# NVIDIA/tensorrt-laboratory

Hardware: AMD Instinct MI355X
Metric: inferences/sec (higher is better)
Workload: dtype fp16; 1 GPU; model=resnet50, global_batch=8, batch_per_gpu=8, image=224, contexts=3, parallelism=dp1

## Files before the change

### csrc/kernels/conv.hip

```cpp
#include "conv_igemm.h"

namespace trtlab {

size_t conv_scratch_bytes(int Nb, int H, int W, int C, int Cout, int KH,
                          int KW, int sh, int sw, int ph, int pw) {
  int OH = (H + 2 * ph - KH) / sh + 1;
  int OW = (W + 2 * pw - KW) / sw + 1;
  int M = Nb * OH * OW;
  int K = (int)round_up(KH * KW * C, 64);
  TileCfg cfg = pick_tile(M, Cout);
  long tiles = cdiv(M, cfg.bm) * cdiv(Cout, cfg.bn);
  int splitk = pick_splitk(tiles, K >> 6);
  if (splitk == 1) return 0;
  return (size_t)tiles * splitk * cfg.bm * cfg.bn * 4;
}

template <typename T, int CM, bool DEEP, int BM = 64>
__global__ __launch_bounds__(256) void bottleneck_tail_kernel(
    const T* __restrict__ in, const T* __restrict__ W1,
    const T* __restrict__ W2, T* __restrict__ out,
    const float* __restrict__ s1, const float* __restrict__ b1,
    const float* __restrict__ s2, const float* __restrict__ b2,
    const T* __restrict__ residual, const T* __restrict__ zero_page,
    const ConvParams p, int Co) {
  constexpr int BNC = 64;
  constexpr int NB1 = CM / BNC;
  constexpr int kABytes = BM * 128;
  constexpr int kBuf = (BM + BNC) * 128;
  constexpr int NBUF = DEEP ? 4 : 2;
  constexpr int kT2 = CM / 64;
  constexpr int kTBlk = BM * 128;
  constexpr int kTBytes = kT2 * kTBlk;
  constexpr int kSmem =
      (NBUF * kBuf > kTBytes + 8192) ? NBUF * kBuf : kTBytes + 8192;
  __shared__ __attribute__((aligned(16))) char smem[kSmem];
  uint32_t lds0 = (uint32_t)(uintptr_t)&smem[0];

  uint32_t tile = xcd_swizzle(blockIdx.x, gridDim.x);
  int m0 = (int)tile * BM;
  const int tid = threadIdx.x;
  const int lane = tid & 63;
  const int wave = tid >> 6;
  const int wr = wave >> 1;
  const int wc = wave & 1;

  typename Mfma16x16x32<T>::accv acc1[NB1][BM / 32][BNC / 32];
#pragma unroll
  for (int c = 0; c < NB1; ++c)
#pragma unroll
    for (int i = 0; i < BM / 32; ++i)
#pragma unroll
      for (int j = 0; j < BNC / 32; ++j) acc1[c][i][j] = {0, 0, 0, 0};

  const int ktiles = p.K / kTileElems<T>;
  const TapRows<BM> rows = tap_rows_init<T, BM>(p, m0, tid);
  for (int nc = 0; nc < NB1; ++nc) {
    TapCursor tap = tap_cursor_init<T>(p, 0);
    auto stage1 = [&](int t, int slot) {
      uint32_t base = lds0 + slot * kBuf;
      stage_conv_a_tap<T, BM>(in, zero_page, p, rows, tap, base, tid);
      stage_tile<T, BNC, true>(W1 + (int64_t)nc * BNC * p.K +
                             (int64_t)t * kTileElems<T>,
                         p.K, nc * BNC, CM, base + kABytes, tid);
    };
    if constexpr (DEEP) {
      constexpr int G = BM / 32 + BNC / 32;
      for (int i = 0; i < 3 && i < ktiles; ++i) stage1(i, i);
      for (int t = 0; t < ktiles; ++t) {
        int ahead = ktiles - 1 - t;
        if (ahead > 2) ahead = 2;
        wait_tiles_inflight<G>(ahead);
        __builtin_amdgcn_s_barrier();
        if (t + 3 < ktiles) stage1(t + 3, (t + 3) & 3);
        const char* As = &smem[(t & 3) * kBuf];
        mfma_tile<T, BM, BNC, true>(As, As + kABytes, lane, wr, wc, acc1[nc]);
      }
      asm volatile("s_waitcnt vmcnt(0)" ::: "memory");
      __syncthreads();
    } else {
      stage1(0, 0);
      asm volatile("s_waitcnt vmcnt(0)" ::: "memory");
      __syncthreads();
      int cur = 0;
      for (int t = 0; t < ktiles; ++t) {
        if (t + 1 < ktiles) stage1(t + 1, cur ^ 1);
        const char* As = &smem[cur * kBuf];
        mfma_tile<T, BM, BNC, true>(As, As + kABytes, lane, wr, wc, acc1[nc]);
        asm volatile("s_waitcnt vmcnt(0)" ::: "memory");
        __syncthreads();
        cur ^= 1;
      }
    }
  }

  static_assert(BNC == 64 && sizeof(T) == 2, "one 16-B chunk per lane");
#pragma unroll
  for (int nc = 0; nc < NB1; ++nc) {
    const int col0 = nc * BNC + wc * (BNC / 2) + (lane >> 4) * 8;
    float sc[8], bi[8];
#pragma unroll
    for (int c = 0; c < 8; ++c) {
      sc[c] = s1[col0 + c];
      bi[c] = b1[col0 + c];
    }
#pragma unroll
    for (int i = 0; i < BM / 32; ++i) {
      uint32_t row = (uint32_t)(wr * (BM / 2) + i * 16 + (lane & 15));
      __attribute__((aligned(16))) T o[8];
#pragma unroll
      for (int j = 0; j < BNC / 32; ++j)
#pragma unroll
        for (int r = 0; r < 4; ++r)
          o[4 * j + r] = (T)fmaxf(
              (float)acc1[nc][i][j][r] * sc[4 * j + r] + bi[4 * j + r], 0.0f);
      uint32_t kb = (uint32_t)(col0 & 63) * (uint32_t)sizeof(T);
      uint32_t off = (uint32_t)(col0 >> 6) * (uint32_t)kTBlk + (row << 7) +
                     (kb ^ ((row & 7) << 4));
      i32x4 t;
      __builtin_memcpy(&t, o, 16);
      *(i32x4*)(smem + off) = t;
    }
  }
  __syncthreads();

  const char* Tlds = smem;
  char* B2s = smem + kTBytes;
  for (int c2 = 0; c2 < Co / 64; ++c2) {
#pragma unroll
    for (int t = 0; t < kT2; ++t)
      stage_tile<T, 64, true>(W2 + (int64_t)c2 * 64 * CM + t * kTileElems<T>, CM,
                        c2 * 64, Co, (uint32_t)(uintptr_t)(B2s + t * 8192),
                        tid);
    asm volatile("s_waitcnt vmcnt(0)" ::: "memory");
    __syncthreads();
    typename Mfma16x16x32<T>::accv acc2[BM / 32][2];
#pragma unroll
    for (int i = 0; i < BM / 32; ++i)
#pragma unroll
      for (int j = 0; j < 2; ++j) acc2[i][j] = {0, 0, 0, 0};
#pragma unroll
    for (int t = 0; t < kT2; ++t)
      mfma_tile<T, BM, 64, true>(Tlds + t * kTBlk, B2s + t * 8192, lane, wr, wc,
                           acc2);
    store_epilogue<T, Epi::kScaleBiasAddRelu, BM, 64>(
        acc2, out, Co, m0, c2 * 64, p.M, Co, s2, b2, residual, p.res_scale,
        lane, wr, wc);
    __syncthreads();
  }
}

void launch_bottleneck_tail(int dtype, const void* in, const void* W1,
                            const void* W2, void* out, const float* s1,
                            const float* b1, const float* s2, const float* b2,
                            const void* residual, const void* zero_page,
                            int Nb, int H, int W, int Cm, int Co,
                            hipStream_t stream) {
  if (dtype != 0)
    throw std::runtime_error("bottleneck_tail: fp16 only");
  if (Cm != 64 && Cm != 128)
    throw std::runtime_error("bottleneck_tail: Cm must be 64 or 128");
  if (Co % 64 != 0) throw std::runtime_error("bottleneck_tail: Co % 64");
  if (!tap_offsets_fit((int64_t)Nb * H * W * Cm * 2))
    throw std::runtime_error("bottleneck_tail: input must be under 2 GiB");
  ConvParams p;
  p.res_scale = 1.0f;
  p.Nb = Nb; p.H = H; p.W = W; p.C = Cm;
  p.Cout = Cm; p.KH = 3; p.KW = 3;
  p.sh = 1; p.sw = 1; p.ph = 1; p.pw = 1;
  p.OH = H; p.OW = W;
  p.M = Nb * H * W;
  p.Kreal = 9 * Cm;
  p.K = p.Kreal;
  p.d_ohw = make_fastdiv((uint32_t)(p.OH * p.OW));
  p.d_ow = make_fastdiv((uint32_t)p.OW);
  p.d_c = make_fastdiv((uint32_t)Cm);
  p.d_kw = make_fastdiv((uint32_t)p.KW);
  int bm = (cdiv(p.M, 64) >= 256) ? 64 : 32;
  dim3 grid((unsigned)cdiv(p.M, bm));
  bool deep = want_deep_pipe(grid.x, p.K / 64);
  auto go = [&](auto cm, auto dp, auto bmv) {
    constexpr int CMv = decltype(cm)::value;
    constexpr bool DPv = decltype(dp)::value;
    constexpr int BMv = decltype(bmv)::value;
    hipLaunchKernelGGL((bottleneck_tail_kernel<_Float16, CMv, DPv, BMv>),
                       grid, dim3(256), 0, stream, (const _Float16*)in,
                       (const _Float16*)W1, (const _Float16*)W2,
                       (_Float16*)out, s1, b1, s2, b2,
                       (const _Float16*)residual, (const _Float16*)zero_page,
                       p, Co);
  };
  auto c64 = std::integral_constant<int, 64>{};
  auto c128 = std::integral_constant<int, 128>{};
  auto b64 = std::integral_constant<int, 64>{};
  auto b32 = std::integral_constant<int, 32>{};
  if (Cm == 64) {
    if (bm == 64) { deep ? go(c64, std::true_type{}, b64)
                         : go(c64, std::false_type{}, b64); }
    else { deep ? go(c64, std::true_type{}, b32)
                : go(c64, std::false_type{}, b32); }
  } else {
// ... 63 lines not shown
```

### csrc/kernels/conv_igemm.h

```cpp
#pragma once
#include "gemm_common.h"

namespace trtlab {

struct ConvParams {
  int Nb, H, W, C;
  int Cout, KH, KW;
  int OH, OW;
  int sh, sw, ph, pw;
  int M;
  int K;
  int Kreal;
  float res_scale;
  FastDiv d_ohw, d_ow, d_c, d_kw;
};

template <typename T, int ROWS>
__device__ __forceinline__ void stage_conv_a(
    const T* __restrict__ in, const T* __restrict__ zero_page,
    const ConvParams p, int m0, int k0, uint32_t lds_base, int tid) {
#pragma unroll
  for (int c = 0; c < ROWS / 32; ++c) {
    uint32_t pbyte = c * 4096 + tid * 16;
    uint32_t row = pbyte >> 7;
// ... 115 lines not shown
void launch_splitk_reduce(int dtype, const float* scratch, void* C,
                          const float* scale, const float* bias,
                          const void* residual, float res_scale, int M, int N,
                          int64_t ldc, int tiles_m, int tiles_n, int splitk,
                          int bm, int bn, int epi, hipStream_t stream);

template <typename T, Epi E, int BM, int BN, bool SPLIT, int NBUF,
          bool TAP = false>
__global__ __launch_bounds__(256) void conv_igemm_kernel(
    const T* __restrict__ in, const T* __restrict__ Wt, T* __restrict__ out,
    const float* __restrict__ scale, const float* __restrict__ bias,
    const T* __restrict__ residual, const T* __restrict__ zero_page,
    const ConvParams p, int tiles_n, float* __restrict__ scratch, int splitk,
    int ktper) {
  constexpr int kABytes = BM * 128;
  constexpr int kBuf = (BM + BN) * 128;

  uint32_t bid = xcd_swizzle(blockIdx.x, gridDim.x);
  uint32_t tile = SPLIT ? bid / splitk : bid;
  int m0 = (int)(tile / tiles_n) * BM;
  int n0 = (int)(tile % tiles_n) * BN;

  __shared__ __attribute__((aligned(16))) char smem[NBUF * kBuf];
  uint32_t lds0 = (uint32_t)(uintptr_t)&smem[0];

  const int tid = threadIdx.x;
  const int lane = tid & 63;
  const int wave = tid >> 6;
  const int wr = wave >> 1;
  const int wc = wave & 1;

  typename Mfma16x16x32<T>::accv acc[BM / 32][BN / 32];
#pragma unroll
  for (int i = 0; i < BM / 32; ++i)
#pragma unroll
    for (int j = 0; j < BN / 32; ++j) acc[i][j] = {0, 0, 0, 0};

  constexpr int KT = kTileElems<T>;
  const int ktiles = p.K / KT;
  int kt0 = 0, kt1 = ktiles;
  if constexpr (SPLIT) {
    int slice = bid % splitk;
    kt0 = slice * ktper;
    kt1 = min(ktiles, kt0 + ktper);
  }

  TapRows<TAP ? BM : 32> rows;
  TapCursor tap;
  if constexpr (TAP) {
    rows = tap_rows_init<T, BM>(p, m0, tid);
    tap = tap_cursor_init<T>(p, kt0);
  }

  auto stage = [&](int t, int slot) {
    uint32_t base = lds0 + slot * kBuf;
    if constexpr (TAP)
      stage_conv_a_tap<T, BM>(in, zero_page, p, rows, tap, base, tid);
    else
      stage_conv_a<T, BM>(in, zero_page, p, m0, t * KT, base, tid);
    stage_tile<T, BN, true>(Wt + (int64_t)n0 * p.K + (int64_t)t * KT, p.K, n0,
                            p.Cout, base + kABytes, tid);
  };

  if constexpr (NBUF == 4) {
    constexpr int G = BM / 32 + BN / 32;
    for (int i = 0; i < 3 && kt0 + i < kt1; ++i) stage(kt0 + i, i);
    for (int t = kt0; t < kt1; ++t) {
      int ahead = kt1 - 1 - t;
      if (ahead > 2) ahead = 2;
      wait_tiles_inflight<G>(ahead);
      __builtin_amdgcn_s_barrier();
      if (t + 3 < kt1) stage(t + 3, (t + 3 - kt0) & 3);
      const char* As = &smem[((t - kt0) & 3) * kBuf];
      mfma_tile<T, BM, BN, true>(As, As + kABytes, lane, wr, wc, acc);
    }
  } else {
    stage(kt0, 0);
    asm volatile("s_waitcnt vmcnt(0)" ::: "memory");
    __syncthreads();
    int cur = 0;
    for (int t = kt0; t < kt1; ++t) {
      if (t + 1 < kt1) stage(t + 1, cur ^ 1);
      const char* As = &smem[cur * kBuf];
      mfma_tile<T, BM, BN, true>(As, As + kABytes, lane, wr, wc, acc);
      asm volatile("s_waitcnt vmcnt(0)" ::: "memory");
      __syncthreads();
      cur ^= 1;
    }
  }

  if constexpr (SPLIT) {
    store_splitk<T, BM, BN>(acc, scratch + (int64_t)bid * BM * BN, lane, wr,
                            wc);
  } else {
    store_epilogue<T, E, BM, BN>(acc, out, p.Cout, m0, n0, p.M, p.Cout, scale,
                                 bias, residual, p.res_scale, lane, wr, wc);
  }
}

static inline bool tap_offsets_fit(int64_t input_bytes) {
  return input_bytes < ((int64_t)1 << 31);
}

template <typename T, Epi E>
__global__ __launch_bounds__(256) void conv_smallk_kernel(
    const T* __restrict__ A, const T* __restrict__ Bw, T* __restrict__ C,
    const float* __restrict__ scale, const float* __restrict__ bias,
    const T* __restrict__ residual, int M, int N, int K, float res_scale,
    int tiles_n) {
  using MF = Mfma16x16x32<T>;
  uint32_t blk = xcd_swizzle(blockIdx.x, gridDim.x);
  int m0 = (int)(blk / tiles_n) * 64, n0 = (int)(blk % tiles_n) * 64;
  int lane = threadIdx.x & 63, wave = threadIdx.x >> 6;
  int arow = m0 + wave * 16 + (lane & 15);
  if (arow >= M) arow = M - 1;
  constexpr int kEps = MF::kStepBytes / (int)sizeof(T);
  constexpr int kFe = MF::kFragBytes / (int)sizeof(T);
  constexpr int kSteps = 128 / MF::kStepBytes;
  f32x4 acc[1][4];
#pragma unroll
  for (int f = 0; f < 4; ++f) acc[0][f] = {0.f, 0.f, 0.f, 0.f};
#pragma unroll
  for (int s = 0; s < kSteps; ++s) {
    int kb = s * kEps + (lane >> 4) * kFe;
    typename MF::frag af =
        *(const typename MF::frag*)(A + (int64_t)arow * K + kb);
#pragma unroll
    for (int f = 0; f < 4; ++f) {
      int brow = n0 + (int)chan_of_frag_row<64>(f * 16 + (lane & 15));
      if (brow >= N) brow = N - 1;
      typename MF::frag bf =
          *(const typename MF::frag*)(Bw + (int64_t)brow * K + kb);
      acc[0][f] = MF::run(bf, af, acc[0][f]);
    }
  }
  store_chan_runs<E>(acc, C, (int64_t)N, m0 + wave * 16 + (lane & 15),
                     n0 + (lane >> 4) * 16, M, N, scale, bias, residual,
                     res_scale, 1.0f);
}

template <typename T>
void launch_conv2d_t(const void* in, const void* Wt, void* out,
                            const float* scale, const float* bias,
                            const void* residual, const void* zero_page,
                            const ConvParams& p, int epi, hipStream_t stream,
                            int tile, float* scratch, int staging) {
  if constexpr (sizeof(T) == 2) {
  if (p.KH == 1 && p.KW == 1 && p.sh == 1 && p.sw == 1 &&
      p.ph == 0 && p.pw == 0 && p.Kreal == p.K && p.K == kTileElems<T> &&
      cdiv(p.M, 64) * cdiv(p.Cout, 64) <= 384) {
    dim3 grid((unsigned)(cdiv(p.M, 64) * cdiv(p.Cout, 64)));
    int tn = (int)cdiv(p.Cout, 64);
    epi_dispatch(epi, [&](auto e) {
      constexpr Epi EE = decltype(e)::value;
      hipLaunchKernelGGL((conv_smallk_kernel<T, EE>), grid, dim3(256), 0,
                         stream, (const T*)in, (const T*)Wt, (T*)out, scale,
                         bias, (const T*)residual, p.M, p.Cout, p.K,
                         p.res_scale, tn);
// ... 80 lines not shown
```

### csrc/kernels/gemm.hip

```cpp
#include "gemm_common.h"

namespace trtlab {

void launch_splitk_reduce(int dtype, const float* scratch, void* C,
                          const float* scale, const float* bias,
                          const void* residual, float res_scale, int M, int N,
                          int64_t ldc, int tiles_m, int tiles_n, int splitk,
                          int bm, int bn, int epi, hipStream_t stream);

template <typename T, typename OT, Epi E, int BM, int BN, bool SPLIT,
          int NBUF>
__global__ __launch_bounds__(256) void gemm_bt_kernel(
    const T* __restrict__ A, const T* __restrict__ B, OT* __restrict__ C,
    const float* __restrict__ scale, const float* __restrict__ bias,
    const OT* __restrict__ residual, float res_scale, float out_scale,
    int M, int N, int K, int64_t lda, int64_t ldb, int64_t ldc, int tiles_n,
    float* __restrict__ scratch, int splitk, int ktper) {
  constexpr int kABytes = BM * 128;
  constexpr int kBuf = (BM + BN) * 128;

  uint32_t bid = xcd_swizzle(blockIdx.x, gridDim.x);
  uint32_t tile = SPLIT ? bid / splitk : bid;
  int m0 = (int)(tile / tiles_n) * BM;
  int n0 = (int)(tile % tiles_n) * BN;

  constexpr int KT = kTileElems<T>;
  const int ktiles = K / KT;
  int kt0 = 0, kt1 = ktiles;
  if constexpr (SPLIT) {
    int slice = bid % splitk;
    kt0 = slice * ktper;
    kt1 = min(ktiles, kt0 + ktper);
  }

  __shared__ __attribute__((aligned(16))) char smem[NBUF * kBuf];
  uint32_t lds0 = (uint32_t)(uintptr_t)&smem[0];

  const int tid = threadIdx.x;
  const int lane = tid & 63;
  const int wave = tid >> 6;
  const int wr = wave >> 1;
  const int wc = wave & 1;

  typename Mfma16x16x32<T>::accv acc[BM / 32][BN / 32];
#pragma unroll
  for (int i = 0; i < BM / 32; ++i)
#pragma unroll
    for (int j = 0; j < BN / 32; ++j) acc[i][j] = {0, 0, 0, 0};

  auto stage = [&](int t, int slot) {
    uint32_t base = lds0 + slot * kBuf;
    stage_tile<T, BM>(A + (int64_t)m0 * lda + (int64_t)t * KT, lda, m0, M,
                      base, tid);
    stage_tile<T, BN, true>(B + (int64_t)n0 * ldb + (int64_t)t * KT, ldb, n0,
                            N, base + kABytes, tid);
  };

  if constexpr (NBUF == 4) {
    constexpr int G = BM / 32 + BN / 32;
    for (int i = 0; i < 3 && kt0 + i < kt1; ++i) stage(kt0 + i, i);
    for (int t = kt0; t < kt1; ++t) {
      int ahead = kt1 - 1 - t;
      if (ahead > 2) ahead = 2;
      wait_tiles_inflight<G>(ahead);
      __builtin_amdgcn_s_barrier();
      if (t + 3 < kt1) stage(t + 3, (t + 3 - kt0) & 3);
      const char* As = &smem[((t - kt0) & 3) * kBuf];
      mfma_tile<T, BM, BN, true>(As, As + kABytes, lane, wr, wc, acc);
    }
  } else if constexpr (NBUF == 3) {
    constexpr int G = BM / 32 + BN / 32;
    stage(kt0, 0);
    if (kt0 + 1 < kt1) stage(kt0 + 1, 1);
    for (int t = kt0; t < kt1; ++t) {
      int ahead = kt1 - 1 - t;
      if (ahead > 1) ahead = 1;
      wait_tiles_inflight<G>(ahead);
      __builtin_amdgcn_s_barrier();
      if (t + 2 < kt1) stage(t + 2, (t + 2 - kt0) % 3);
      const char* As = &smem[((t - kt0) % 3) * kBuf];
      mfma_tile<T, BM, BN, true>(As, As + kABytes, lane, wr, wc, acc);
    }
  } else {
    stage(kt0, 0);
    asm volatile("s_waitcnt vmcnt(0)" ::: "memory");
    __syncthreads();
    int cur = 0;
    for (int t = kt0; t < kt1; ++t) {
      if (t + 1 < kt1) stage(t + 1, cur ^ 1);
      const char* As = &smem[cur * kBuf];
      mfma_tile<T, BM, BN, true>(As, As + kABytes, lane, wr, wc, acc);
      asm volatile("s_waitcnt vmcnt(0)" ::: "memory");
      __syncthreads();
      cur ^= 1;
    }
  }

  if constexpr (SPLIT) {
    store_splitk<T, BM, BN>(acc, scratch + (int64_t)bid * BM * BN, lane, wr,
                            wc);
  } else {
    store_epilogue<T, E, BM, BN, OT>(acc, C, ldc, m0, n0, M, N, scale, bias,
                                     residual, res_scale, lane, wr, wc,
                                     out_scale);
  }
}

size_t gemm_scratch_bytes(int M, int N, int K) {
  TileCfg cfg = pick_tile(M, N);
  long tiles = cdiv(M, cfg.bm) * cdiv(N, cfg.bn);
  int splitk = pick_splitk_gemm(tiles, K >> 6);
  if (splitk == 1) return 0;
  return (size_t)tiles * splitk * cfg.bm * cfg.bn * 4;
}

template <typename T, typename OT = T>
static void launch_gemm_bt_t(const void* A, const void* B, void* C,
                             const float* scale, const float* bias,
                             const void* residual, float res_scale,
                             float out_scale, int M, int N, int K,
                             int64_t lda, int64_t ldb, int64_t ldc, int epi,
                             hipStream_t stream, int tile, float* scratch) {
  TileCfg cfg = tile ? tile_from_code(tile) : pick_tile(M, N);
  int tiles_m = (int)cdiv(M, cfg.bm);
  int tiles_n = (int)cdiv(N, cfg.bn);
  long tiles = (long)tiles_m * tiles_n;
  int ktiles = K / kTileElems<T>;
  if (cfg.bm == 256) {
    dim3 grid5((unsigned)tiles);
    epi_dispatch(epi, [&](auto e) {
      constexpr Epi EE = decltype(e)::value;
      hipLaunchKernelGGL((gemm_bt_kernel<T, OT, EE, 256, 128, false, 3>),
                         grid5, dim3(256), 0, stream, (const T*)A,
                         (const T*)B, (OT*)C, scale, bias,
                         (const OT*)residual, res_scale, out_scale, M, N, K,
                         lda, ldb, ldc, tiles_n, (float*)nullptr, 1, ktiles);
    });
    return;
  }
  int splitk = (!tile && scratch) ? pick_splitk_gemm(tiles, ktiles) : 1;
  dim3 block(256);
  int out_dtype = std::is_same<OT, _Float16>::value
                      ? 0
                      : (std::is_same<OT, __bf16>::value
                             ? 1
                             : (std::is_same<OT, int8_t>::value ? 2 : 3));
  if (splitk > 1) {
    int ktper = (int)cdiv(ktiles, splitk);
    dim3 grid((unsigned)(tiles * splitk));
    bool deep = want_deep_pipe(tiles * splitk, ktper);
    tile_dispatch(cfg, [&](auto bm, auto bn) {
      constexpr int BM = decltype(bm)::value;
      constexpr int BN = decltype(bn)::value;
      if (deep)
        hipLaunchKernelGGL((gemm_bt_kernel<T, OT, Epi::kNone, BM, BN, true, 4>),
                           grid, block, 0, stream, (const T*)A, (const T*)B,
                           (OT*)C, scale, bias, (const OT*)residual,
// ... 75 lines not shown
```

### csrc/kernels/gemm_common.h

```cpp
#pragma once
#include <hip/hip_fp8.h>

#include "../common.h"

namespace trtlab {

enum class Epi : int {
  kNone = 0,
  kBias = 1,
  kBiasRelu = 2,
  kBiasGelu = 3,
  kScaleBias = 4,
  kScaleBiasRelu = 5,
  kScaleBiasAddRelu = 6,
  kScaleBiasGelu = 7,
};

__device__ __forceinline__ float gelu_tanh(float x) {
  const float k0 = 0.7978845608028654f;
  const float k1 = 0.044715f;
  float u = k0 * (x + k1 * x * x * x);
  return 0.5f * x * (1.0f + tanhf(u));
}

// ... 104 lines not shown
    uint32_t p = c * 4096 + tid * 16;
    uint32_t row = p >> 7;
    uint32_t kb = (p & 127) ^ ((row & 7) << 4);
    uint32_t srow = row;
    if constexpr (CHAN_RUNS) {
      constexpr uint32_t kHalf = ROWS / 2;
      srow = (row & ~(kHalf - 1)) + chan_of_frag_row<kHalf>(row & (kHalf - 1));
    }
    int r = row0 + (int)srow;
    r = (r < 0) ? 0 : (r >= nrows ? nrows - 1 : r);
    const char* g = (const char*)src +
                    ((int64_t)r - row0) * stride_elems * (int64_t)sizeof(T) +
                    kb;
    glds16(g, lds_base + p);
  }
}

template <typename T>
__device__ __forceinline__ typename Mfma16x16x32<T>::frag read_frag(
    const char* lds, uint32_t row, uint32_t kbyte) {
  uint32_t off = (row << 7) + (kbyte ^ ((row & 7) << 4));
  return *(const typename Mfma16x16x32<T>::frag*)(lds + off);
}

template <typename T, int BM, int BN, bool CHAN_RUNS = false>
__device__ __forceinline__ void mfma_tile(
    const char* As, const char* Bs, int lane, int wr, int wc,
    typename Mfma16x16x32<T>::accv (&acc)[BM / 32][BN / 32]) {
  using MF = Mfma16x16x32<T>;
  constexpr int MFr = BM / 32, NFr = BN / 32;
  constexpr int kSteps = 128 / MF::kStepBytes;
#pragma unroll
  for (int ks = 0; ks < kSteps; ++ks) {
    typename MF::frag af[MFr], bf[NFr];
    uint32_t kbyte = ks * MF::kStepBytes + ((lane >> 4) * MF::kFragBytes);
#pragma unroll
    for (int f = 0; f < MFr; ++f)
      af[f] = read_frag<T>(As, wr * (BM / 2) + f * 16 + (lane & 15), kbyte);
#pragma unroll
    for (int f = 0; f < NFr; ++f)
      bf[f] = read_frag<T>(Bs, wc * (BN / 2) + f * 16 + (lane & 15), kbyte);
#pragma unroll
    for (int i = 0; i < MFr; ++i)
#pragma unroll
      for (int j = 0; j < NFr; ++j) {
        if constexpr (CHAN_RUNS)
          acc[i][j] = MF::run(bf[j], af[i], acc[i][j]);
        else
          acc[i][j] = MF::run(af[i], bf[j], acc[i][j]);
      }
  }
}

template <int BYTES>
struct RawVec;
template <>
struct RawVec<4> { using type = int; };
template <>
struct RawVec<8> { using type = i32x2; };
template <>
struct RawVec<16> { using type = i32x4; };

template <Epi E>
constexpr bool kEpiHasScale =
    E == Epi::kScaleBias || E == Epi::kScaleBiasRelu ||
    E == Epi::kScaleBiasAddRelu || E == Epi::kScaleBiasGelu;

template <Epi E, typename AccV, int MF, int NF, typename OT>
__device__ __forceinline__ void store_chan_runs(
    AccV (&acc)[MF][NF], OT* __restrict__ C, int64_t ldc, int row0, int col0,
    int M, int N, const float* __restrict__ scale,
    const float* __restrict__ bias, const OT* __restrict__ residual,
    float res_scale, float out_scale) {
  constexpr bool kRes = E == Epi::kScaleBiasAddRelu;
  constexpr int CH = 4 * NF;
  constexpr int VE = (16 / (int)sizeof(OT) < CH) ? 16 / (int)sizeof(OT) : CH;
  constexpr int VB = VE * (int)sizeof(OT);
  constexpr int JV = VE / 4;
  using RV = typename RawVec<VB>::type;

  uintptr_t mis = (uintptr_t)C | (uintptr_t)(ldc * (int64_t)sizeof(OT));
  if constexpr (kRes) mis |= (uintptr_t)residual;
  uintptr_t mis16 = 0;
  if constexpr (kEpiHasScale<E>) mis16 |= (uintptr_t)scale;
  if constexpr (E != Epi::kNone) mis16 |= (uintptr_t)bias;
  const bool vec =
      col0 + CH <= N && (mis & (VB - 1)) == 0 && (mis16 & 15) == 0;

  if (vec) {
#pragma unroll
    for (int v = 0; v < CH / VE; ++v) {
      const int colv = col0 + v * VE;
      f32x4 sc[JV], bi[JV];
#pragma unroll
      for (int jj = 0; jj < JV; ++jj) {
        sc[jj] = {1.0f, 1.0f, 1.0f, 1.0f};
        bi[jj] = {0.0f, 0.0f, 0.0f, 0.0f};
        if constexpr (kEpiHasScale<E>)
          sc[jj] = *(const f32x4*)(scale + colv + 4 * jj);
        if constexpr (E != Epi::kNone)
          bi[jj] = *(const f32x4*)(bias + colv + 4 * jj);
      }
#pragma unroll
      for (int i = 0; i < MF; ++i) {
        int row = row0 + i * 16;
        if (row >= M) continue;
        int64_t off = (int64_t)row * ldc + colv;
        __attribute__((aligned(16))) OT rs[VE];
        __attribute__((aligned(16))) OT o[VE];
        if constexpr (kRes) {
          RV t = *(const RV*)(residual + off);
          __builtin_memcpy(rs, &t, VB);
        }
#pragma unroll
        for (int jj = 0; jj < JV; ++jj)
#pragma unroll
          for (int r = 0; r < 4; ++r) {
            float res = 0.0f;
            if constexpr (kRes) res = (float)rs[4 * jj + r] * res_scale;
            float val = apply_epi<E>((float)acc[i][v * JV + jj][r], sc[jj][r],
                                     bi[jj][r], res);
            o[4 * jj + r] = store_cast<OT>(val * out_scale);
            if constexpr (E == Epi::kScaleBias &&
                          std::is_same<OT, _Float16>::value)
              asm("" : "+v"(o[4 * jj + r]));
          }
        RV t;
        __builtin_memcpy(&t, o, VB);
        *(RV*)(C + off) = t;
      }
    }
  } else {
#pragma unroll
    for (int j = 0; j < NF; ++j) {
#pragma unroll
      for (int r = 0; r < 4; ++r) {
        int col = col0 + 4 * j + r;
        if (col >= N) continue;
        float sc = 1.0f, bi = 0.0f;
        if constexpr (kEpiHasScale<E>) sc = scale[col];
        if constexpr (E != Epi::kNone) bi = bias[col];
#pragma unroll
        for (int i = 0; i < MF; ++i) {
          int row = row0 + i * 16;
          if (row >= M) continue;
          float res = 0.0f;
          if constexpr (kRes)
            res = (float)residual[(int64_t)row * ldc + col] * res_scale;
          float val = apply_epi<E>((float)acc[i][j][r], sc, bi, res);
          C[(int64_t)row * ldc + col] = store_cast<OT>(val * out_scale);
        }
      }
    }
  }
}

template <typename T, Epi E, int BM, int BN, typename OT = T>
__device__ __forceinline__ void store_epilogue(
    typename Mfma16x16x32<T>::accv (&acc)[BM / 32][BN / 32],
    OT* __restrict__ C, int64_t ldc, int m0, int n0, int M, int N,
    const float* __restrict__ scale, const float* __restrict__ bias,
    const OT* __restrict__ residual, float res_scale, int lane, int wr,
    int wc, float out_scale = 1.0f) {
  int row0 = m0 + wr * (BM / 2) + (lane & 15);
  int col0 = n0 + wc * (BN / 2) + (lane >> 4) * (BN / 8);
  store_chan_runs<E>(acc, C, ldc, row0, col0, M, N, scale, bias, residual,
                     res_scale, out_scale);
}

template <int G>
__device__ __forceinline__ void wait_tiles_inflight(int ahead) {
  static_assert(2 * G <= 63, "vmcnt is a 6-bit counter");
  if (ahead >= 2)
    asm volatile("s_waitcnt vmcnt(%0)" ::"n"(2 * G) : "memory");
  else if (ahead == 1)
    asm volatile("s_waitcnt vmcnt(%0)" ::"n"(G) : "memory");
  else
    asm volatile("s_waitcnt vmcnt(0)" ::: "memory");
}

inline bool want_deep_pipe(long blocks, int ktiles) {
  static const long gate = [] {
    const char* e = getenv("TRTLAB_DEEP_GATE");
    return e ? atol(e) : 384L;
  }();
  return blocks < gate && ktiles >= 2;
}

template <typename T, int BM, int BN>
__device__ __forceinline__ void store_splitk(
    typename Mfma16x16x32<T>::accv (&acc)[BM / 32][BN / 32],
    float* __restrict__ slab, int lane, int wr, int wc) {
  const int col0 = wc * (BN / 2) + (lane >> 4) * (BN / 8);
#pragma unroll
  for (int i = 0; i < BM / 32; ++i) {
    int row = wr * (BM / 2) + i * 16 + (lane & 15);
#pragma unroll
    for (int j = 0; j < BN / 32; ++j) {
      f32x4 v = {(float)acc[i][j][0], (float)acc[i][j][1],
                 (float)acc[i][j][2], (float)acc[i][j][3]};
      *(f32x4*)(slab + row * BN + col0 + 4 * j) = v;
    }
  }
}

inline int pick_splitk(long blocks, int ktiles) {
  if (blocks > 144 || ktiles < 24) return 1;
  int splitk = 1;
  while (blocks * splitk < 256 && ktiles / (splitk * 2) >= 4 && splitk < 8)
    splitk *= 2;
  return splitk;
}

inline int pick_splitk_gemm(long blocks, int ktiles) {
  if (blocks > 144 || ktiles < 8) return 1;
  int splitk = 1;
  while (blocks * splitk < 256 && ktiles / (splitk * 2) >= 3 && splitk < 8)
    splitk *= 2;
// ... 61 lines not shown
```

### csrc/kernels/pool.hip

```cpp
#include <hip/hip_fp8.h>

#include "../common.h"

namespace trtlab {

template <typename T>
__global__ void maxpool2d_kernel(const T* __restrict__ in, T* __restrict__ out,
                                 int Nb, int H, int W, int C, int KH, int KW,
                                 int sh, int sw, int ph, int pw, int OH,
                                 int OW) {
  int cg = C >> 3;
  int64_t total = (int64_t)Nb * OH * OW * cg;
  for (int64_t idx = (int64_t)blockIdx.x * blockDim.x + threadIdx.x;
       idx < total; idx += (int64_t)gridDim.x * blockDim.x) {
    int c8 = (int)(idx % cg);
    int64_t q = idx / cg;
    int ow = (int)(q % OW);
    q /= OW;
    int oh = (int)(q % OH);
    int n = (int)(q / OH);
    float best[8];
#pragma unroll
    for (int j = 0; j < 8; ++j) best[j] = -3.0e38f;
    for (int kh = 0; kh < KH; ++kh) {
// ... 45 lines not shown
        int iw = ow * sw - pw + kw;
        if ((unsigned)iw >= (unsigned)W) continue;
        const T* p = in + ((((int64_t)n * H + ih) * W + iw) * C) + c8 * 8;
        T tmp[8];
        if constexpr (sizeof(T) == 2) {
          *(short4v*)&tmp[0] = *(const short4v*)p;
          *(short4v*)&tmp[4] = *(const short4v*)(p + 4);
        } else {
          *(uint2*)&tmp[0] = *(const uint2*)p;
        }
#pragma unroll
        for (int j = 0; j < 8; ++j) acc[j] += (float)tmp[j];
        ++cnt;
      }
    }
    float inv = cnt ? 1.0f / cnt : 0.0f;
    T* o = out + ((((int64_t)n * OH + oh) * OW + ow) * C) + c8 * 8;
#pragma unroll
    for (int j = 0; j < 8; ++j) o[j] = (T)(acc[j] * inv);
  }
}

void launch_avgpool2d(int dtype, const void* in, void* out, int Nb, int H,
                      int W, int C, int KH, int KW, int sh, int sw, int ph,
                      int pw, hipStream_t stream) {
  if (C % 8 != 0) throw std::runtime_error("avgpool2d: C % 8 != 0");
  int OH = (H + 2 * ph - KH) / sh + 1;
  int OW = (W + 2 * pw - KW) / sw + 1;
  int64_t total = (int64_t)Nb * OH * OW * (C / 8);
  int blocks = (int)std::min<int64_t>(cdiv(total, 256), 2048);
  if (dtype == 0)
    hipLaunchKernelGGL((avgpool2d_kernel<_Float16>), dim3(blocks), dim3(256),
                       0, stream, (const _Float16*)in, (_Float16*)out, Nb, H,
                       W, C, KH, KW, sh, sw, ph, pw, OH, OW);
  else if (dtype == 1)
    hipLaunchKernelGGL((avgpool2d_kernel<__bf16>), dim3(blocks), dim3(256), 0,
                       stream, (const __bf16*)in, (__bf16*)out, Nb, H, W, C,
                       KH, KW, sh, sw, ph, pw, OH, OW);
  else
    throw std::runtime_error("avgpool2d: fp16/bf16 only");
}

template <typename T>
__global__ void gavgpool_kernel(const T* __restrict__ in, T* __restrict__ out,
                                int Nb, int HW, int C) {
  int cg = C >> 3;
  int total = Nb * cg;
  for (int idx = blockIdx.x * blockDim.x + threadIdx.x; idx < total;
       idx += gridDim.x * blockDim.x) {
    int c8 = idx % cg;
    int n = idx / cg;
    float acc[8] = {0, 0, 0, 0, 0, 0, 0, 0};
    const T* base = in + ((int64_t)n * HW * C) + c8 * 8;
    for (int i = 0; i < HW; ++i) {
      short4v v0 = *(const short4v*)(base + (int64_t)i * C);
      short4v v1 = *(const short4v*)(base + (int64_t)i * C + 4);
#pragma unroll
      for (int j = 0; j < 4; ++j) {
        acc[j] += (float)((const T*)&v0)[j];
        acc[4 + j] += (float)((const T*)&v1)[j];
      }
    }
    float inv = 1.0f / (float)HW;
    T* o = out + (int64_t)n * C + c8 * 8;
#pragma unroll
    for (int j = 0; j < 8; ++j) o[j] = (T)(acc[j] * inv);
  }
}

template <typename T>
static void launch_maxpool2d_t(const void* in, void* out, int Nb, int H, int W,
                               int C, int KH, int KW, int sh, int sw, int ph,
                               int pw, hipStream_t stream) {
  int OH = (H + 2 * ph - KH) / sh + 1;
  int OW = (W + 2 * pw - KW) / sw + 1;
  int64_t total = (int64_t)Nb * OH * OW * (C / 8);
  int blocks = (int)std::min<int64_t>(cdiv(total, 256), 2048);
  hipLaunchKernelGGL((maxpool2d_kernel<T>), dim3(blocks), dim3(256), 0, stream,
                     (const T*)in, (T*)out, Nb, H, W, C, KH, KW, sh, sw, ph,
                     pw, OH, OW);
}

void launch_maxpool2d(int dtype, const void* in, void* out, int Nb, int H,
                      int W, int C, int KH, int KW, int sh, int sw, int ph,
                      int pw, hipStream_t stream) {
  if (C % 8 != 0) throw std::runtime_error("maxpool2d: C % 8 != 0");
  if (dtype == 0)
    launch_maxpool2d_t<_Float16>(in, out, Nb, H, W, C, KH, KW, sh, sw, ph, pw, stream);
  else if (dtype == 1)
    launch_maxpool2d_t<__bf16>(in, out, Nb, H, W, C, KH, KW, sh, sw, ph, pw, stream);
  else if (dtype == 2)
    launch_maxpool2d_t<int8_t>(in, out, Nb, H, W, C, KH, KW, sh, sw, ph, pw, stream);
  else
    launch_maxpool2d_t<__hip_fp8_e4m3>(in, out, Nb, H, W, C, KH, KW, sh, sw,
                                       ph, pw, stream);
}

void launch_gavgpool(int dtype, const void* in, void* out, int Nb, int HW,
                     int C, hipStream_t stream) {
  if (C % 8 != 0) throw std::runtime_error("gavgpool: C % 8 != 0");
  int total = Nb * (C / 8);
  int blocks = std::min((int)cdiv(total, 256), 2048);
  if (blocks < 1) blocks = 1;
  if (dtype == 0)
    hipLaunchKernelGGL((gavgpool_kernel<_Float16>), dim3(blocks), dim3(256), 0,
                       stream, (const _Float16*)in, (_Float16*)out, Nb, HW, C);
  else
// ... 6 lines not shown
```

Measured before the change: 27350 inf/s.

## Prefetch epilogue operands, double-buffer bottleneck W2 tiles, batch gavgpool loads

Splits the GEMM and conv epilogues into a load phase and an apply/store phase. Scale, bias and residual loads can now be issued at kernel entry, or one vector at a time, so their latency overlaps the main loop. The fused bottleneck tail now double-buffers its second-stage weight tiles and prefetches the next chunk's epilogue operands while the current chunk computes. Occupancy hints are added to several kernels through launch_bounds, and the global average pool unrolls its loads in batches of seven. The cost is more registers held across the main loop, which could reduce occupancy or cause spills.

```diff
diff --git a/csrc/kernels/conv.hip b/csrc/kernels/conv.hip
--- a/csrc/kernels/conv.hip
+++ b/csrc/kernels/conv.hip
@@ -16,7 +16,8 @@
 }
 
 template <typename T, int CM, bool DEEP, int BM = 64>
-__global__ __launch_bounds__(256) void bottleneck_tail_kernel(
+__global__ __launch_bounds__(256, (CM == 128 && !DEEP && BM == 32) ? 6 : 1)
+void bottleneck_tail_kernel(
     const T* __restrict__ in, const T* __restrict__ W1,
     const T* __restrict__ W2, T* __restrict__ out,
     const float* __restrict__ s1, const float* __restrict__ b1,
@@ -51,6 +52,19 @@
     for (int i = 0; i < BM / 32; ++i)
 #pragma unroll
       for (int j = 0; j < BNC / 32; ++j) acc1[c][i][j] = {0, 0, 0, 0};
+
+  static_assert(BNC == 64 && sizeof(T) == 2, "one 16-B chunk per lane");
+  constexpr bool kS1AtEntry = NB1 == 1;
+  float sc1[NB1][8], bi1[NB1][8];
+  auto load_s1 = [&](int nc) {
+    const int col0 = nc * BNC + wc * (BNC / 2) + (lane >> 4) * 8;
+#pragma unroll
+    for (int c = 0; c < 8; ++c) {
+      sc1[nc][c] = s1[col0 + c];
+      bi1[nc][c] = b1[col0 + c];
+    }
+  };
+  if constexpr (kS1AtEntry) load_s1(0);
 
   const int ktiles = p.K / kTileElems<T>;
   const TapRows<BM> rows = tap_rows_init<T, BM>(p, m0, tid);
@@ -93,16 +107,34 @@
     }
   }
 
-  static_assert(BNC == 64 && sizeof(T) == 2, "one 16-B chunk per lane");
+  constexpr int kB2 = kT2 * 8192;
+  constexpr int NSLOT = (kTBytes + 2 * kB2 <= kSmem) ? 2 : 1;
+  constexpr Epi E2 = Epi::kScaleBiasAddRelu;
+  using Ops2 = EpiOperands<E2, BM / 32, 2, T>;
+  char* B2s = smem + kTBytes;
+  const int nchunks = Co / 64;
+  auto stage2 = [&](int c2, int slot) {
+#pragma unroll
+    for (int t = 0; t < kT2; ++t)
+      stage_tile<T, 64, true>(
+          W2 + (int64_t)c2 * 64 * CM + t * kTileElems<T>, CM, c2 * 64, Co,
+          (uint32_t)(uintptr_t)(B2s + slot * kB2 + t * 8192), tid);
+  };
+  auto load2 = [&](Ops2& o, int c2) {
+    int row0, col0;
+    tile_lane_origin<BM, 64>(m0, c2 * 64, lane, wr, wc, row0, col0);
+    epi_load<true, true>(o, out, Co, row0, col0, p.M, Co, s2, b2, residual);
+  };
+  Ops2 cur;
+  stage2(0, 0);
+  if constexpr (kS1AtEntry && NSLOT == 2) load2(cur, 0);
+
 #pragma unroll
   for (int nc = 0; nc < NB1; ++nc) {
     const int col0 = nc * BNC + wc * (BNC / 2) + (lane >> 4) * 8;
-    float sc[8], bi[8];
-#pragma unroll
-    for (int c = 0; c < 8; ++c) {
-      sc[c] = s1[col0 + c];
-      bi[c] = b1[col0 + c];
-    }
+    if constexpr (!kS1AtEntry) load_s1(nc);
+    const float(&sc)[8] = sc1[nc];
+    const float(&bi)[8] = bi1[nc];
 #pragma unroll
     for (int i = 0; i < BM / 32; ++i) {
       uint32_t row = (uint32_t)(wr * (BM / 2) + i * 16 + (lane & 15));
@@ -121,31 +153,45 @@
       *(i32x4*)(smem + off) = t;
     }
   }
+  if constexpr (!kS1AtEntry && NSLOT == 2) load2(cur, 0);
+  asm volatile("s_waitcnt vmcnt(0)" ::: "memory");
   __syncthreads();
 
   const char* Tlds = smem;
-  char* B2s = smem + kTBytes;
-  for (int c2 = 0; c2 < Co / 64; ++c2) {
+  for (int c2 = 0; c2 < nchunks; ++c2) {
+    const bool more = c2 + 1 < nchunks;
+    const int slot = NSLOT == 2 ? (c2 & 1) : 0;
+    typename Mfma16x16x32<T>::accv acc2[BM / 32][2];
+#pragma unroll
+    for (int i = 0; i < BM / 32; ++i)
+#pragma unroll
+      for (int j = 0; j < 2; ++j) acc2[i][j] = {0, 0, 0, 0};
 #pragma unroll
     for (int t = 0; t < kT2; ++t)
-      stage_tile<T, 64, true>(W2 + (int64_t)c2 * 64 * CM + t * kTileElems<T>, CM,
-                        c2 * 64, Co, (uint32_t)(uintptr_t)(B2s + t * 8192),
-                        tid);
-    asm volatile("s_waitcnt vmcnt(0)" ::: "memory");
-    __syncthreads();
-    typename Mfma16x16x32<T>::accv acc2[BM / 32][2];
-#pragma unroll
-    for (int i = 0; i < BM / 32; ++i)
-#pragma unroll
-      for (int j = 0; j < 2; ++j) acc2[i][j] = {0, 0, 0, 0};
-#pragma unroll
-    for (int t = 0; t < kT2; ++t)
-      mfma_tile<T, BM, 64, true>(Tlds + t * kTBlk, B2s + t * 8192, lane, wr, wc,
-                           acc2);
-    store_epilogue<T, Epi::kScaleBiasAddRelu, BM, 64>(
-        acc2, out, Co, m0, c2 * 64, p.M, Co, s2, b2, residual, p.res_scale,
-        lane, wr, wc);
-    __syncthreads();
+      mfma_tile<T, BM, 64, true>(Tlds + t * kTBlk,
+                                 B2s + slot * kB2 + t * 8192, lane, wr, wc,
+                                 acc2);
+    int row0, col0;
+    tile_lane_origin<BM, 64>(m0, c2 * 64, lane, wr, wc, row0, col0);
+    if constexpr (NSLOT == 2) {
+      epi_apply_store<E2>(acc2, cur, out, Co, row0, col0, p.M, Co, s2, b2,
+                          residual, p.res_scale, 1.0f);
+      if (!more) break;
+      stage2(c2 + 1, (c2 + 1) & 1);
+      load2(cur, c2 + 1);
+    } else {
+      store_chan_runs<E2>(acc2, out, Co, row0, col0, p.M, Co, s2, b2,
+                          residual, p.res_scale, 1.0f);
+      if (!more) break;
+      asm volatile("" ::: "memory");
+      __builtin_amdgcn_s_barrier();
+      asm volatile("" ::: "memory");
+      stage2(c2 + 1, 0);
+    }
+    asm volatile("" ::: "memory");
+    __builtin_amdgcn_s_waitcnt(kWaitVmcnt0);
+    __builtin_amdgcn_s_barrier();
+    asm volatile("" ::: "memory");
   }
 }
 
diff --git a/csrc/kernels/conv_igemm.h b/csrc/kernels/conv_igemm.h
--- a/csrc/kernels/conv_igemm.h
+++ b/csrc/kernels/conv_igemm.h
@@ -191,6 +191,18 @@
     tap = tap_cursor_init<T>(p, kt0);
   }
 
+  constexpr EpiPrefetch kPre =
+      SPLIT ? EpiPrefetch::kAfterLoop
+            : epi_prefetch_mode<E, BM, BN, (int)sizeof(T)>();
+  EpiOperands<E, BM / 32, BN / 32, T> ops;
+  int row0, col0;
+  tile_lane_origin<BM, BN>(m0, n0, lane, wr, wc, row0, col0);
+  if constexpr (kPre == EpiPrefetch::kEntry ||
+                kPre == EpiPrefetch::kResidualAtEntry)
+    epi_load<kPre == EpiPrefetch::kEntry, true>(ops, out, p.Cout, row0, col0,
+                                                p.M, p.Cout, scale, bias,
+                                                residual);
+
   auto stage = [&](int t, int slot) {
     uint32_t base = lds0 + slot * kBuf;
     if constexpr (TAP)
@@ -232,8 +244,16 @@
     store_splitk<T, BM, BN>(acc, scratch + (int64_t)bid * BM * BN, lane, wr,
                             wc);
   } else {
-    store_epilogue<T, E, BM, BN>(acc, out, p.Cout, m0, n0, p.M, p.Cout, scale,
-                                 bias, residual, p.res_scale, lane, wr, wc);
+    if constexpr (kPre == EpiPrefetch::kByVector) {
+      store_chan_runs_by_vector<E>(acc, out, p.Cout, row0, col0, p.M, p.Cout,
+                                   scale, bias, residual, p.res_scale, 1.0f);
+    } else {
+      if constexpr (kPre != EpiPrefetch::kEntry)
+        epi_load<true, kPre == EpiPrefetch::kAfterLoop>(
+            ops, out, p.Cout, row0, col0, p.M, p.Cout, scale, bias, residual);
+      epi_apply_store<E>(acc, ops, out, p.Cout, row0, col0, p.M, p.Cout,
+                         scale, bias, residual, p.res_scale, 1.0f);
+    }
   }
 }
 
@@ -242,7 +262,8 @@
 }
 
 template <typename T, Epi E>
-__global__ __launch_bounds__(256) void conv_smallk_kernel(
+__global__ __launch_bounds__(256, E == Epi::kScaleBiasAddRelu ? 6 : 1)
+void conv_smallk_kernel(
     const T* __restrict__ A, const T* __restrict__ Bw, T* __restrict__ C,
     const float* __restrict__ scale, const float* __restrict__ bias,
     const T* __restrict__ residual, int M, int N, int K, float res_scale,
diff --git a/csrc/kernels/gemm.hip b/csrc/kernels/gemm.hip
--- a/csrc/kernels/gemm.hip
+++ b/csrc/kernels/gemm.hip
@@ -10,7 +10,10 @@
 
 template <typename T, typename OT, Epi E, int BM, int BN, bool SPLIT,
           int NBUF>
-__global__ __launch_bounds__(256) void gemm_bt_kernel(
+__global__ __launch_bounds__(
+    256, (BM == 128 && BN == 128 && NBUF == 2 && sizeof(OT) == 1 &&
+          E == Epi::kScaleBiasAddRelu) ? 2 : 1)
+void gemm_bt_kernel(
     const T* __restrict__ A, const T* __restrict__ B, OT* __restrict__ C,
     const float* __restrict__ scale, const float* __restrict__ bias,
     const OT* __restrict__ residual, float res_scale, float out_scale,
@@ -47,6 +50,17 @@
   for (int i = 0; i < BM / 32; ++i)
 #pragma unroll
     for (int j = 0; j < BN / 32; ++j) acc[i][j] = {0, 0, 0, 0};
+
+  constexpr EpiPrefetch kPre =
+      SPLIT ? EpiPrefetch::kAfterLoop
+            : epi_prefetch_mode<E, BM, BN, (int)sizeof(OT)>();
+  EpiOperands<E, BM / 32, BN / 32, OT> ops;
+  int row0, col0;
+  tile_lane_origin<BM, BN>(m0, n0, lane, wr, wc, row0, col0);
+  if constexpr (kPre == EpiPrefetch::kEntry ||
+                kPre == EpiPrefetch::kResidualAtEntry)
+    epi_load<kPre == EpiPrefetch::kEntry, true>(ops, C, ldc, row0, col0, M, N,
+                                                scale, bias, residual);
 
   auto stage = [&](int t, int slot) {
     uint32_t base = lds0 + slot * kBuf;
@@ -100,9 +114,16 @@
     store_splitk<T, BM, BN>(acc, scratch + (int64_t)bid * BM * BN, lane, wr,
                             wc);
   } else {
-    store_epilogue<T, E, BM, BN, OT>(acc, C, ldc, m0, n0, M, N, scale, bias,
-                                     residual, res_scale, lane, wr, wc,
-                                     out_scale);
+    if constexpr (kPre == EpiPrefetch::kByVector) {
+      store_chan_runs_by_vector<E>(acc, C, ldc, row0, col0, M, N, scale, bias,
+                                   residual, res_scale, out_scale);
+    } else {
+      if constexpr (kPre != EpiPrefetch::kEntry)
+        epi_load<true, kPre == EpiPrefetch::kAfterLoop>(
+            ops, C, ldc, row0, col0, M, N, scale, bias, residual);
+      epi_apply_store<E>(acc, ops, C, ldc, row0, col0, M, N, scale, bias,
+                         residual, res_scale, out_scale);
+    }
   }
 }
 
diff --git a/csrc/kernels/gemm_common.h b/csrc/kernels/gemm_common.h
--- a/csrc/kernels/gemm_common.h
+++ b/csrc/kernels/gemm_common.h
@@ -180,6 +180,8 @@
   }
 }
 
+constexpr int kWaitVmcnt0 = 0x0F70;
+
 template <int BYTES>
 struct RawVec;
 template <>
@@ -194,71 +196,105 @@
     E == Epi::kScaleBias || E == Epi::kScaleBiasRelu ||
     E == Epi::kScaleBiasAddRelu || E == Epi::kScaleBiasGelu;
 
-template <Epi E, typename AccV, int MF, int NF, typename OT>
-__device__ __forceinline__ void store_chan_runs(
-    AccV (&acc)[MF][NF], OT* __restrict__ C, int64_t ldc, int row0, int col0,
-    int M, int N, const float* __restrict__ scale,
-    const float* __restrict__ bias, const OT* __restrict__ residual,
-    float res_scale, float out_scale) {
+template <int NF, typename OT>
+struct EpiGeom {
+  static constexpr int CH = 4 * NF;
+  static constexpr int VE =
+      (16 / (int)sizeof(OT) < CH) ? 16 / (int)sizeof(OT) : CH;
+  static constexpr int VB = VE * (int)sizeof(OT);
+  static constexpr int JV = VE / 4;
+  static constexpr int NV = CH / VE;
+  using RV = typename RawVec<VB>::type;
+};
+
+template <Epi E, int MF, int NF, typename OT>
+struct EpiOperands {
+  using G = EpiGeom<NF, OT>;
+  f32x4 sc[G::NV][G::JV], bi[G::NV][G::JV];
+  typename G::RV rs[G::NV][MF];
+  bool vec;
+};
+
+template <bool SB, bool RES, int V0 = 0, int V1 = -1, Epi E, int MF, int NF,
+          typename OT>
+__device__ __forceinline__ void epi_load(
+    EpiOperands<E, MF, NF, OT>& ops, const OT* __restrict__ C, int64_t ldc,
+    int row0, int col0, int M, int N, const float* __restrict__ scale,
+    const float* __restrict__ bias, const OT* __restrict__ residual) {
+  using G = EpiGeom<NF, OT>;
   constexpr bool kRes = E == Epi::kScaleBiasAddRelu;
-  constexpr int CH = 4 * NF;
-  constexpr int VE = (16 / (int)sizeof(OT) < CH) ? 16 / (int)sizeof(OT) : CH;
-  constexpr int VB = VE * (int)sizeof(OT);
-  constexpr int JV = VE / 4;
-  using RV = typename RawVec<VB>::type;
-
   uintptr_t mis = (uintptr_t)C | (uintptr_t)(ldc * (int64_t)sizeof(OT));
   if constexpr (kRes) mis |= (uintptr_t)residual;
   uintptr_t mis16 = 0;
   if constexpr (kEpiHasScale<E>) mis16 |= (uintptr_t)scale;
   if constexpr (E != Epi::kNone) mis16 |= (uintptr_t)bias;
-  const bool vec =
-      col0 + CH <= N && (mis & (VB - 1)) == 0 && (mis16 & 15) == 0;
-
-  if (vec) {
-#pragma unroll
-    for (int v = 0; v < CH / VE; ++v) {
-      const int colv = col0 + v * VE;
-      f32x4 sc[JV], bi[JV];
-#pragma unroll
-      for (int jj = 0; jj < JV; ++jj) {
-        sc[jj] = {1.0f, 1.0f, 1.0f, 1.0f};
-        bi[jj] = {0.0f, 0.0f, 0.0f, 0.0f};
+  ops.vec =
+      col0 + G::CH <= N && (mis & (G::VB - 1)) == 0 && (mis16 & 15) == 0;
+  if (!ops.vec) return;
+#pragma unroll
+  for (int v = V0; v < (V1 < 0 ? G::NV : V1); ++v) {
+    const int colv = col0 + v * G::VE;
+    if constexpr (SB) {
+#pragma unroll
+      for (int jj = 0; jj < G::JV; ++jj) {
+        ops.sc[v][jj] = {1.0f, 1.0f, 1.0f, 1.0f};
+        ops.bi[v][jj] = {0.0f, 0.0f, 0.0f, 0.0f};
         if constexpr (kEpiHasScale<E>)
-          sc[jj] = *(const f32x4*)(scale + colv + 4 * jj);
+          ops.sc[v][jj] = *(const f32x4*)(scale + colv + 4 * jj);
         if constexpr (E != Epi::kNone)
-          bi[jj] = *(const f32x4*)(bias + colv + 4 * jj);
+          ops.bi[v][jj] = *(const f32x4*)(bias + colv + 4 * jj);
       }
+    }
+    if constexpr (RES && kRes) {
+#pragma unroll
+      for (int i = 0; i < MF; ++i) {
+        int row = min(row0 + i * 16, M - 1);
+        ops.rs[v][i] =
+            *(const typename G::RV*)(residual + (int64_t)row * ldc + colv);
+      }
+    }
+  }
+}
+
+template <Epi E, int V0 = 0, int V1 = -1, typename AccV, int MF, int NF,
+          typename OT>
+__device__ __forceinline__ void epi_apply_store(
+    AccV (&acc)[MF][NF], const EpiOperands<E, MF, NF, OT>& ops,
+    OT* __restrict__ C, int64_t ldc, int row0, int col0, int M, int N,
+    const float* __restrict__ scale, const float* __restrict__ bias,
+    const OT* __restrict__ residual, float res_scale, float out_scale) {
+  using G = EpiGeom<NF, OT>;
+  constexpr bool kRes = E == Epi::kScaleBiasAddRelu;
+  if (ops.vec) {
+    if constexpr (E != Epi::kNone) __builtin_amdgcn_s_waitcnt(kWaitVmcnt0);
+#pragma unroll
+    for (int v = V0; v < (V1 < 0 ? G::NV : V1); ++v) {
+      const int colv = col0 + v * G::VE;
 #pragma unroll
       for (int i = 0; i < MF; ++i) {
         int row = row0 + i * 16;
-        if (row >= M) continue;
-        int64_t off = (int64_t)row * ldc + colv;
-        __attribute__((aligned(16))) OT rs[VE];
-        __attribute__((aligned(16))) OT o[VE];
-        if constexpr (kRes) {
-          RV t = *(const RV*)(residual + off);
-          __builtin_memcpy(rs, &t, VB);
-        }
-#pragma unroll
-        for (int jj = 0; jj < JV; ++jj)
+        __attribute__((aligned(16))) OT rs[G::VE];
+        __attribute__((aligned(16))) OT o[G::VE];
+        if constexpr (kRes) __builtin_memcpy(rs, &ops.rs[v][i], G::VB);
+#pragma unroll
+        for (int jj = 0; jj < G::JV; ++jj)
 #pragma unroll
           for (int r = 0; r < 4; ++r) {
             float res = 0.0f;
             if constexpr (kRes) res = (float)rs[4 * jj + r] * res_scale;
-            float val = apply_epi<E>((float)acc[i][v * JV + jj][r], sc[jj][r],
-                                     bi[jj][r], res);
+            float val = apply_epi<E>((float)acc[i][v * G::JV + jj][r],
+                                     ops.sc[v][jj][r], ops.bi[v][jj][r], res);
             o[4 * jj + r] = store_cast<OT>(val * out_scale);
             if constexpr (E == Epi::kScaleBias &&
                           std::is_same<OT, _Float16>::value)
               asm("" : "+v"(o[4 * jj + r]));
           }
-        RV t;
-        __builtin_memcpy(&t, o, VB);
-        *(RV*)(C + off) = t;
+        typename G::RV t;
+        __builtin_memcpy(&t, o, G::VB);
+        if (row < M) *(typename G::RV*)(C + (int64_t)row * ldc + colv) = t;
       }
     }
-  } else {
+  } else if (V0 == 0) {
 #pragma unroll
     for (int j = 0; j < NF; ++j) {
 #pragma unroll
@@ -280,7 +316,61 @@
         }
       }
     }
-  }
+    __builtin_amdgcn_s_waitcnt(kWaitVmcnt0);
+  }
+}
+
+template <Epi E, typename AccV, int MF, int NF, typename OT>
+__device__ __forceinline__ void store_chan_runs(
+    AccV (&acc)[MF][NF], OT* __restrict__ C, int64_t ldc, int row0, int col0,
+    int M, int N, const float* __restrict__ scale,
+    const float* __restrict__ bias, const OT* __restrict__ residual,
+    float res_scale, float out_scale) {
+  EpiOperands<E, MF, NF, OT> ops;
+  epi_load<true, true>(ops, C, ldc, row0, col0, M, N, scale, bias, residual);
+  epi_apply_store<E>(acc, ops, C, ldc, row0, col0, M, N, scale, bias,
+                     residual, res_scale, out_scale);
+}
+
+template <Epi E, typename AccV, int MF, int NF, typename OT>
+__device__ __forceinline__ void store_chan_runs_by_vector(
+    AccV (&acc)[MF][NF], OT* __restrict__ C, int64_t ldc, int row0, int col0,
+    int M, int N, const float* __restrict__ scale,
+    const float* __restrict__ bias, const OT* __restrict__ residual,
+    float res_scale, float out_scale) {
+  EpiOperands<E, MF, NF, OT> ops;
+  epi_load<true, true, 0, 1>(ops, C, ldc, row0, col0, M, N, scale, bias,
+                             residual);
+  epi_apply_store<E, 0, 1>(acc, ops, C, ldc, row0, col0, M, N, scale, bias,
+                           residual, res_scale, out_scale);
+  if constexpr (EpiGeom<NF, OT>::NV > 1) {
+    epi_load<true, true, 1>(ops, C, ldc, row0, col0, M, N, scale, bias,
+                            residual);
+    epi_apply_store<E, 1>(acc, ops, C, ldc, row0, col0, M, N, scale, bias,
+                          residual, res_scale, out_scale);
+  }
+}
+
+enum class EpiPrefetch : int {
+  kByVector = -1, kAfterLoop = 0, kResidualAtEntry = 1, kEntry = 2
+};
+template <Epi E, int BM, int BN, int OB>
+constexpr EpiPrefetch epi_prefetch_mode() {
+  constexpr bool kRes = E == Epi::kScaleBiasAddRelu;
+  if (E == Epi::kNone) return EpiPrefetch::kAfterLoop;
+  if (BM == 256) return EpiPrefetch::kAfterLoop;
+  if (BM == 128 && BN == 128 && kRes) return EpiPrefetch::kByVector;
+  if (BM == 64 && BN == 128 && OB == 1 && kRes)
+    return EpiPrefetch::kResidualAtEntry;
+  return EpiPrefetch::kEntry;
+}
+
+template <int BM, int BN>
+__device__ __forceinline__ void tile_lane_origin(int m0, int n0, int lane,
+                                                 int wr, int wc, int& row0,
+                                                 int& col0) {
+  row0 = m0 + wr * (BM / 2) + (lane & 15);
+  col0 = n0 + wc * (BN / 2) + (lane >> 4) * (BN / 8);
 }
 
 template <typename T, Epi E, int BM, int BN, typename OT = T>
@@ -290,8 +380,8 @@
     const float* __restrict__ scale, const float* __restrict__ bias,
     const OT* __restrict__ residual, float res_scale, int lane, int wr,
     int wc, float out_scale = 1.0f) {
-  int row0 = m0 + wr * (BM / 2) + (lane & 15);
-  int col0 = n0 + wc * (BN / 2) + (lane >> 4) * (BN / 8);
+  int row0, col0;
+  tile_lane_origin<BM, BN>(m0, n0, lane, wr, wc, row0, col0);
   store_chan_runs<E>(acc, C, ldc, row0, col0, M, N, scale, bias, residual,
                      res_scale, out_scale);
 }
diff --git a/csrc/kernels/pool.hip b/csrc/kernels/pool.hip
--- a/csrc/kernels/pool.hip
+++ b/csrc/kernels/pool.hip
@@ -121,7 +121,24 @@
     int n = idx / cg;
     float acc[8] = {0, 0, 0, 0, 0, 0, 0, 0};
     const T* base = in + ((int64_t)n * HW * C) + c8 * 8;
-    for (int i = 0; i < HW; ++i) {
+    constexpr int kBatch = 7;
+    int i = 0;
+    for (; i + kBatch <= HW; i += kBatch) {
+      short4v v0[kBatch], v1[kBatch];
+#pragma unroll
+      for (int u = 0; u < kBatch; ++u) {
+        v0[u] = *(const short4v*)(base + (int64_t)(i + u) * C);
+        v1[u] = *(const short4v*)(base + (int64_t)(i + u) * C + 4);
+      }
+#pragma unroll
+      for (int u = 0; u < kBatch; ++u)
+#pragma unroll
+        for (int j = 0; j < 4; ++j) {
+          acc[j] += (float)((const T*)&v0[u])[j];
+          acc[4 + j] += (float)((const T*)&v1[u])[j];
+        }
+    }
+    for (; i < HW; ++i) {
       short4v v0 = *(const short4v*)(base + (int64_t)i * C);
       short4v v1 = *(const short4v*)(base + (int64_t)i * C + 4);
 #pragma unroll
```

Measured after the change: 27530 inf/s (median of 5 runs). Within noise of the previous version (+0.7%).
